# pennucci/PulsePortraiture

Hardware: AMD Instinct MI355X
Metric: subint_fits_per_sec (higher is better)
Workload: dtype f64

## Files before the change

### pulseportraiture_amd/csrc/pp_common.h

```cpp
#pragma once
#include <hip/hip_runtime.h>
#include <stdint.h>
#include <type_traits>

namespace pp {

#define PP_DCONST 4149.377593360996
#define PP_TWO_PI 6.283185307179586476925286766559
#define PP_LN10 2.302585092994045684017991454684

typedef double2 cplx;

__device__ __forceinline__ cplx cmul(cplx a, cplx b) {
    return make_double2(fma(a.x, b.x, -a.y * b.y), fma(a.x, b.y, a.y * b.x));
}
__device__ __forceinline__ cplx cmulc(cplx a, cplx b) {
    return make_double2(fma(a.x, b.x, a.y * b.y), fma(a.y, b.x, -a.x * b.y));
}
__device__ __forceinline__ cplx cadd(cplx a, cplx b) { return make_double2(a.x + b.x, a.y + b.y); }
__device__ __forceinline__ cplx csub(cplx a, cplx b) { return make_double2(a.x - b.x, a.y - b.y); }
__device__ __forceinline__ cplx cmul_mi(cplx a) { return make_double2(a.y, -a.x); }
__device__ __forceinline__ double cnorm(cplx a) { return fma(a.x, a.x, a.y * a.y); }

template <typename T>
__device__ __forceinline__ const T* as_global(const T* p) {
    typedef const T __attribute__((address_space(1)))* gp_t;
    return (const T*)(gp_t)(uintptr_t)p;
}

template <typename T>
__device__ __forceinline__ T load_uniform(const T* p) {
    typedef const T __attribute__((address_space(4)))* cp_t;
    return *(cp_t)(uintptr_t)p;
}

__device__ __forceinline__ double rn_pin(double r) { asm volatile("" : "+v"(r)); return r; }
__device__ __forceinline__ double mul_rn(double a, double b) { return rn_pin(a * b); }
__device__ __forceinline__ double add_rn(double a, double b) { return rn_pin(a + b); }
__device__ __forceinline__ double sub_rn(double a, double b) { return rn_pin(a - b); }

__device__ __forceinline__ double recip_ge1(double x) {
    double y = __builtin_amdgcn_rcp(x);
    y = fma(fma(-x, y, 1.0), y, y);
    y = fma(fma(-x, y, 1.0), y, y);
    return (x < 1e300) ? y : 0.0;
}

template <bool SC>
__device__ __forceinline__ double kconst(double v) {
    if (SC) asm volatile("" : "+s"(v));
    return v;
}
template <bool SC = false>
__device__ __forceinline__ void sincos_turns(double t, double* sn, double* cs) {
    const double q = rint(4.0 * t);
    const double y = fma(-0.25, q, t);
    const double u = y * y;
    double ps = kconst<SC>(0x1.aaec32af93359p-4);
    ps = fma(ps, u, kconst<SC>(-0x1.6fadb9f155744p-1));
    ps = fma(ps, u, kconst<SC>(0x1.e8f434d018d63p+1));
    ps = fma(ps, u, kconst<SC>(-0x1.e3074fde8871fp+3));
    ps = fma(ps, u, kconst<SC>(0x1.50783487ee782p+5));
    ps = fma(ps, u, kconst<SC>(-0x1.32d2cce62bd86p+6));
    ps = fma(ps, u, kconst<SC>(0x1.466bc6775aae2p+6));
    ps = fma(ps, u, kconst<SC>(-0x1.4abbce625be53p+5));
    ps = fma(ps, u, kconst<SC>(0x1.921fb54442d18p+2));
    const double s0 = ps * y;
    double pc = kconst<SC>(0x1.20c62c2f2d7f5p-2);
    pc = fma(pc, u, kconst<SC>(-0x1.b6e24f44b128fp+0));
    pc = fma(pc, u, kconst<SC>(0x1.f9d38a3763cc3p+2));
    pc = fma(pc, u, kconst<SC>(-0x1.a6d1f2a204a8cp+4));
    pc = fma(pc, u, kconst<SC>(0x1.e1f506891babbp+5));
    pc = fma(pc, u, kconst<SC>(-0x1.55d3c7e3cbffap+6));
    pc = fma(pc, u, kconst<SC>(0x1.03c1f081b5ac4p+6));
    pc = fma(pc, u, kconst<SC>(-0x1.3bd3cc9be45dep+4));
    const double c0 = fma(pc, u, 1.0);
    const int qi = (int)q;
    const bool odd = qi & 1;
    const double so = odd ? c0 : s0, co = odd ? s0 : c0;
    *sn = (qi & 2) ? -so : so;
    *cs = ((qi + 1) & 2) ? -co : co;
}

template <bool SC = false>
__device__ __forceinline__ cplx unit_phasor(double k, double phi) {
    double pfrac = phi - rint(phi);
    double prod = k * pfrac;
    double err = fma(k, pfrac, -prod);
    double r = (prod - rint(prod)) + err;
    double s, c;
    sincos_turns<SC>(r, &s, &c);
    return make_double2(c, s);
}

template <int W>
__device__ __forceinline__ double group_sum(double v) {
#pragma unroll
    for (int o = W / 2; o > 0; o >>= 1) v += __shfl_xor(v, o, 64);
    return v;
}
template <int W>
__device__ __forceinline__ double group_max(double v) {
#pragma unroll
    for (int o = W / 2; o > 0; o >>= 1) v = fmax(v, __shfl_xor(v, o, 64));
    return v;
}

__device__ __forceinline__ int wave_reduce16_index(int lane) { return (lane >> 2) & 15; }
template <int NS>
__device__ __forceinline__ double wave_reduce16(const double (&s)[NS], int lane) {
    double t8[8], t4[4], t2[2];
    const bool b5 = lane & 32, b4 = lane & 16, b3 = lane & 8, b2 = lane & 4;
#pragma unroll
    for (int j = 0; j < 8; ++j) {
        const double hi = (j + 8 < NS) ? s[j + 8] : 0.0;
        const double keep = b5 ? hi : s[j], send = b5 ? s[j] : hi;
        t8[j] = keep + __shfl_xor(send, 32, 64);
    }
#pragma unroll
    for (int j = 0; j < 4; ++j) {
        const double keep = b4 ? t8[j + 4] : t8[j], send = b4 ? t8[j] : t8[j + 4];
        t4[j] = keep + __shfl_xor(send, 16, 64);
    }
#pragma unroll
    for (int j = 0; j < 2; ++j) {
        const double keep = b3 ? t4[j + 2] : t4[j], send = b3 ? t4[j] : t4[j + 2];
        t2[j] = keep + __shfl_xor(send, 8, 64);
    }
    const double keep = b2 ? t2[1] : t2[0], send = b2 ? t2[0] : t2[1];
    double v = keep + __shfl_xor(send, 4, 64);
    v += __shfl_xor(v, 2, 64);
    v += __shfl_xor(v, 1, 64);
    return v;
}

template <int NS>
__device__ __forceinline__ double wave_reduce_lds(const double (&s)[NS], int lane, double* buf) {
    static_assert(NS <= 16, "one value per lane quad");
    const int wpos = (lane >> 4) * 17 + (lane & 15);
#pragma unroll
    for (int q = 0; q < NS; ++q) buf[q * 68 + wpos] = s[q];
    const int q = min(lane >> 2, NS - 1), part = lane & 3;
    const double* src = buf + q * 68 + part * 17;
    double v = 0.0;
#pragma unroll
    for (int t = 0; t < 16; ++t) v += src[t];
    v += __shfl_xor(v, 1, 64);
    v += __shfl_xor(v, 2, 64);
    return v;
}
#define PP_WRED_DOUBLES(NS) ((NS) * 68)

template <int NV>
__device__ inline void block_sum(double (&v)[NV], double* scratch) {
    const int lane = threadIdx.x & 63, wid = threadIdx.x >> 6, nw = blockDim.x >> 6;
#pragma unroll
    for (int i = 0; i < NV; ++i) v[i] = group_sum<64>(v[i]);
    __syncthreads();
    if (lane == 0) {
#pragma unroll
        for (int i = 0; i < NV; ++i) scratch[wid * NV + i] = v[i];
    }
    __syncthreads();
#pragma unroll
    for (int i = 0; i < NV; ++i) {
        double s = 0.0;
        for (int w = 0; w < nw; ++w) s += scratch[w * NV + i];
        v[i] = s;
    }
}

template <int NV, int C0>
__device__ __forceinline__ void wave_totals_to(const double (&v)[NV], int lane, double* dst) {
    constexpr int n = (NV - C0) < 16 ? (NV - C0) : 16;
    double part[n];
#pragma unroll
    for (int j = 0; j < n; ++j) part[j] = v[C0 + j];
    const double tot = wave_reduce16<n>(part, lane);
    if ((lane & 3) == 0 && (lane >> 2) < n) dst[C0 + (lane >> 2)] = tot;
    if constexpr (C0 + 16 < NV) wave_totals_to<NV, C0 + 16>(v, lane, dst);
}
// ... 57 lines not shown
```

### pulseportraiture_amd/csrc/pp_kernels.h

```cpp
#pragma once
#include "pp_fft.h"

namespace pp {

struct ModelFftArgs {
    const void* port;
    cplx* mft;
    double* msum;
    double* mmax;
    double* mdc;
    double* msq;
    const cplx* twB;
    int nchan;
};

struct TailArgs;
#define PP_TAIL_LDS_DOUBLES 2176
#define PP_TAIL_CACHE ((PP_TAIL_LDS_DOUBLES - 536) / 4)
__device__ void tail_work(const TailArgs* t, double* lds, int nlds, int tid, int max_tickets);

struct XspecArgs {
    const void* data;
    const cplx* const* mft;
    const cplx* mft0;
    const int* const* ktab;
    const int* kt0;
    const int* slot;
    cplx* X;
    double* sdraw;
    double* noise;
    const cplx* twB;
    int nsub, nchan, Kt;
    int Xs;
    const double* x0;
    const double* P;
    const double* nu_fit;
    const double* freqs; long long freqs_stride;
    double* csum0;
    double* tay;
    const double* ph0;
    const int* act;
    int cstep, coff, nchan_full;
    unsigned* ticket;
    unsigned ticket_base;
    int x_f32;
    const unsigned* mwords;
    const TailArgs* tail;
    int tail_nsub;
};

__device__ __forceinline__ void store_x(const XspecArgs& a, size_t row, int k, const cplx& x) {
    if (a.x_f32) reinterpret_cast<float2*>(a.X)[row * a.Xs + (k - 1)] = make_float2((float)x.x, (float)x.y);
    else a.X[row * a.Xs + (k - 1)] = x;
}

struct FitArgs {
    int nsub, nchan, nbin, M, Kt;
    int Xs;
    int flags[5];
    int log10_tau, option, is_toa, max_iter, scat;
    int method;
    const cplx* X;
    const cplx* const* mft;
    const double* const* msq;
    const double* const* msum;
    const int* const* ktab;
    const int* slot;
    const double* freqs; long long freqs_stride;
    const double* wts;
    const double* sdraw;
    const double* P;
    const double* nu_fit;
    const double* nu_out;
    const double* x0;
    SubState* st;
    double* csum;
    int ncs;
    double* tay;
    double* partial;
    int nchunk, cpc;
    int* nactive;
    double* o_params; double* o_errs; double* o_nu; double* o_cov;
    double* o_chi2; double* o_rchi2; double* o_snr; int* o_nfev; int* o_rc; int* o_npass;
    double* o_scales; double* o_scale_errs; double* o_csnr;
    double* o_f0; double* o_g0; double* o_H0;
    double* o_rec;
    const int* act;
    int nact, nchan_x, cstep, coff;
    double* mdl;
    int use_model;
    double model_tol;
    int model_bet;
    int recentre;
    double* x0w;
    int x_f32;
    const double* xstart;
    int nfev_shadow;
    int solve_cache;
    int tail_fused;
    int x_full;
};

__device__ __forceinline__ int sub_of(const int* act, int j) { return act ? act[j] : j; }

template <typename P>
__device__ __forceinline__ const P* uniform_ptr(const P* p) {
    const unsigned long long u = reinterpret_cast<unsigned long long>(p);
    const unsigned lo = (unsigned)__builtin_amdgcn_readfirstlane((int)(unsigned)u);
    const unsigned hi = (unsigned)__builtin_amdgcn_readfirstlane((int)(unsigned)(u >> 32));
    return as_global(reinterpret_cast<const P*>(((unsigned long long)hi << 32) | (unsigned long long)lo));
}

__device__ __forceinline__ bool channel_lookup(const XspecArgs& a, int ia, int n, int ne, int M, int& n_held,
                                               const cplx*& mrow, int& ktn) {
    if (!a.slot && n == n_held) return false;
    const cplx* m = as_global(a.slot ? a.mft[a.slot[ia]] : a.mft0) + (size_t)ne * M;
    const int k = a.ktab ? as_global(a.slot ? a.ktab[a.slot[ia]] : a.kt0)[ne] : a.Kt;
    mrow = uniform_ptr(m);
    ktn = __builtin_amdgcn_readfirstlane(k);
    n_held = n;
    return true;
}

template <int M, typename Tin>
__global__ __launch_bounds__(FftPlan<M>::T) void k_model_fft(ModelFftArgs a) {
    constexpr int T = FftPlan<M>::T;
    __shared__ cplx lds[FftPlan<M>::LDS_ELEMS];
    __shared__ double red[2 * (T / 64) + 2];
    const int tid = threadIdx.x;
    for (int n = blockIdx.x; n < a.nchan; n += gridDim.x) {
        const Tin* grow = reinterpret_cast<const Tin*>(a.port) + (size_t)n * (2 * M);
        fft_row<M, Tin>(lds, grow, a.twB, tid);
        double s = 0.0, mx = 0.0;
        for (int k = 1 + tid; k <= M; k += T) {
            const cplx d = rfft_harmonic<M>(lds, a.twB, k);
            a.mft[(size_t)n * M + (k - 1)] = d;
            const double p = cnorm(d);
            a.msq[(size_t)n * M + (k - 1)] = p;
            s += p;
            mx = fmax(mx, p);
        }
        s = group_sum<64>(s);
        mx = group_max<64>(mx);
        if (T > 64) {
            if ((tid & 63) == 0) { red[2 * (tid >> 6)] = s; red[2 * (tid >> 6) + 1] = mx; }
            __syncthreads();
            if (tid == 0) {
                s = 0.0; mx = 0.0;
                for (int w = 0; w < T / 64; ++w) { s += red[2 * w]; mx = fmax(mx, red[2 * w + 1]); }
            }
        }
        if (tid == 0) {
            a.msum[n] = s; a.mmax[n] = mx;
            const cplx z0 = lds[0];
            a.mdc[n] = z0.x + z0.y;
        }
        __syncthreads();
    }
}

__global__ void k_model_kcut(const cplx* mft, const double* mmax, int , int M, double eps2,
                             int* kt, int* kmax) {
    const int n = blockIdx.x;
    const double thr = eps2 * mmax[n];
    int last = 0;
    for (int k = 1 + threadIdx.x; k <= M; k += blockDim.x)
        if (cnorm(mft[(size_t)n * M + k - 1]) > thr) last = k;
    for (int o = 32; o > 0; o >>= 1) last = max(last, __shfl_xor(last, o, 64));
    if ((threadIdx.x & 63) == 0) {
        const int v = min(M, max(64, ((last + 63) / 64) * 64));
        kt[n] = v;
// ... 1021 lines not shown
    return rho > 0.15;
}

#define PP_FOR_N3(n_, EXPR)           \
    switch (n_) {                     \
        case 1: { constexpr int N_ = 1; EXPR; } break; \
        case 2: { constexpr int N_ = 2; EXPR; } break; \
        default: { constexpr int N_ = 3; EXPR; } break; \
    }
__device__ __forceinline__ double sel3(double v0, double v1, double v2, int k) { return k == 0 ? v0 : (k == 1 ? v1 : v2); }
template <int N>
__device__ __forceinline__ void gather_sub3(const double (&g)[3], const double (&H)[9], const int (&ix)[3], double (&gs)[N],
                                            double (&Hs)[N * N]) {
#pragma unroll
    for (int r = 0; r < N; ++r) {
        const int k = ix[r];
        gs[r] = sel3(g[0], g[1], g[2], k);
        const double r0 = sel3(H[0], H[3], H[6], k), r1 = sel3(H[1], H[4], H[7], k), r2 = sel3(H[2], H[5], H[8], k);
#pragma unroll
        for (int c = 0; c < N; ++c) Hs[r * N + c] = sel3(r0, r1, r2, ix[c]);
    }
}
template <int N>
__device__ __forceinline__ void scatter_sub3(const double (&p)[N], const int (&ix)[3], double (&p3)[3]) {
#pragma unroll
    for (int j = 0; j < 3; ++j) {
        p3[j] = 0.0;
#pragma unroll
        for (int r = 0; r < N; ++r) if (ix[r] == j) p3[j] = p[r];
    }
}
template <int N>
__device__ __forceinline__ void tr_propose_scipy3(double f, const double (&g)[3], const double (&H)[9], const int (&ix)[3],
                                                  double radius, double (&p3)[3], int& hits, double& pred) {
    double gs[N], Hs[N * N], p[N];
    gather_sub3<N>(g, H, ix, gs, Hs);
    tr_cg_steihaug_scipy<N>(f, gs, Hs, radius, p, &hits);
    pred = f - tr_model_value<N>(f, gs, Hs, p);
    scatter_sub3<N>(p, ix, p3);
}
template <int N>
__device__ __forceinline__ bool newton_propose3(const double (&g)[3], const double (&H)[9], const int (&ix)[3], double (&p3)[3],
                                                double& pred) {
    double gs[N], Hs[N * N], p[N], mg[N], Hp[N];
    gather_sub3<N>(g, H, ix, gs, Hs);
#pragma unroll
    for (int r = 0; r < N; ++r) mg[r] = -gs[r];
    if (!chol_solve<N>(Hs, mg, p)) return false;
#pragma unroll
    for (int r = 0; r < N; ++r) Hp[r] = vdot<N>(Hs + r * N, p);
    pred = -(vdot<N>(gs, p) + 0.5 * vdot<N>(p, Hp));
    scatter_sub3<N>(p, ix, p3);
    return true;
}

__global__ __launch_bounds__(256) void k_eval_moments(FitArgs a) {
    constexpr int LPC = 16;
    const int jx = blockIdx.x, i = sub_of(a.act, jx), chunk = blockIdx.y;
    const SubState& st = a.st[i];
    const int tid = threadIdx.x, g = tid / LPC, l = tid % LPC;
    const double phi = st.xe[0], DM = st.xe[1], GM = st.xe[2];
    const double P = a.P[i];
    const double nuDM = a.nu_fit[i * 3], nuGM = a.nu_fit[i * 3 + 1];
    const double* freqs = a.freqs + (size_t)i * a.freqs_stride;
    const double* wts = a.wts + (size_t)i * a.nchan;
    const int* ktv = a.ktab ? as_global(a.ktab[a.slot ? a.slot[i] : 0]) : nullptr;
    double* tay = a.tay;
    const size_t row0 = (size_t)i * a.nchan;
    const int n0 = chunk * a.cpc, n1 = min(n0 + a.cpc, a.nchan_x);
    const int src = ((tid & 63) & ~(LPC - 1)) | (LPC - 1);
    for (int nn = n0 + g; nn < n1; nn += 256 / LPC) {
        const int n = a.coff + nn * a.cstep;
        const double w = wts[n];
        double p1, p2;
        phase_geom(freqs[n], P, nuDM, nuGM, p1, p2);
        const double phin = phi + DM * p1 + GM * p2;
        cplx e0 = unit_phasor((double)(l + 1), phin);
        const cplx w1 = make_double2(__shfl(e0.x, src, 64), __shfl(e0.y, src, 64));
        const cplx w2 = cmul(w1, w1), w3 = cmul(w2, w1), w4 = cmul(w2, w2);
        const cplx* xrow = a.X + ((size_t)jx * a.nchan_x + nn) * a.Xs;
        const int ktn = ktv ? ktv[n] : a.Kt;
        double s[PP_TSTRIDE];
#pragma unroll
        for (int j = 0; j < PP_TSTRIDE; ++j) s[j] = 0.0;
        double k = (double)(l + 1);
        if (w != 0.0) {
#pragma unroll 1
            for (int jj = l; jj < ktn; jj += 4 * LPC) {
                const cplx zero = make_double2(0.0, 0.0);
                cplx xv[4];
                xv[0] = xrow[jj];
                xv[1] = (jj + LPC < ktn) ? xrow[jj + LPC] : zero;
                xv[2] = (jj + 2 * LPC < ktn) ? xrow[jj + 2 * LPC] : zero;
                xv[3] = (jj + 3 * LPC < ktn) ? xrow[jj + 3 * LPC] : zero;
                cplx ev[4];
                ev[0] = e0; ev[1] = cmul(e0, w1); ev[2] = cmul(e0, w2); ev[3] = cmul(e0, w3);
#pragma unroll
                for (int q = 0; q < 4; ++q) {
                    const cplx z = cmul(xv[q], ev[q]);
                    const double kap = PP_TWO_PI * (k + (double)(q * LPC));
                    const double kap2 = kap * kap;
                    double ur = z.x, ui = z.y * kap;
#pragma unroll
                    for (int j = 0; j <= PP_TJ; j += 2) {
                        s[j] += ur;
                        ur *= kap2;
                        if (j + 1 <= PP_TJ) { s[j + 1] += ui; ui *= kap2; }
                    }
                    static_assert(PP_TJ % 2 == 0, "PP_TJ must be even");
                    double pw = kap;
#pragma unroll
                    for (int j = 0; j < PP_TJ / 2; ++j) pw *= kap2;
                    s[PP_TJ + 1] = fma(pw, fabs(xv[q].x) + fabs(xv[q].y), s[PP_TJ + 1]);
                }
                e0 = cmul(e0, w4);
                k += 4.0 * LPC;
            }
        }
#pragma unroll
        for (int j = 0; j < PP_TSTRIDE; ++j) {
            double v = group_sum<LPC>(s[j]);
            if (j <= PP_TJ && ((j & 3) == 1 || (j & 3) == 2)) v = -v;
            if (l == (j % LPC)) tay[tay_idx(row0 + n, j)] = v;
        }
    }
}

__device__ __forceinline__ void taylor_load(const double* tay, size_t row, double (&t)[PP_TSTRIDE]) {
    static_assert(PP_TSTRIDE % 2 == 0, "rows of the Taylor model are read in pairs");
    const double* tg = tay + tay_idx(row, 0);
#pragma unroll
    for (int j = 0; j < PP_TSTRIDE / 2; ++j) {
        const double2 v = *reinterpret_cast<const double2*>(tg + j * PP_TAY_PAIR_STRIDE);
        t[2 * j] = v.x; t[2 * j + 1] = v.y;
    }
}
__device__ __forceinline__ void taylor_shift_reg(const double (&t)[PP_TSTRIDE], double d, double& A0, double& A1,
                                                 double& A2);
__device__ __forceinline__ void taylor_shift_reg(const double (&t)[PP_TSTRIDE], double d, double& A0, double& A1,
                                                 double& A2) {
    double a0 = 0.0, a1 = 0.0, a2 = 0.0;
#pragma unroll
    for (int j = PP_TJ; j >= 0; --j) {
        a0 = fma(a0, d * (1.0 / (double)(j + 1)), t[j]);
        if (j >= 1) a1 = fma(a1, d * (1.0 / (double)j), t[j]);
        if (j >= 2) a2 = fma(a2, d * (1.0 / (double)(j - 1)), t[j]);
    }
    A0 = a0; A1 = a1; A2 = a2;
}

#define PP_SOLVE_CACHE_MAX 4096
constexpr int PP_SOLVE_PF = 2;
constexpr int PP_TAYLOR_WAVES = 2;
template <int NV, int NVMAX, int NT, int NVW, typename F>
__device__ __forceinline__ void vblock_sum(double (&out)[NV], double* scratch, int& flip, double* mx, int tid, F&& accumulate) {
    static_assert(NV <= NVMAX, "scratch sized for NVMAX values");
    constexpr int NWV = NT / 64, RT = NT / NVW;
    const int lane = tid & 63, rw = tid >> 6;
    double* buf = scratch + flip * NWV * (NVMAX + 1);
    flip ^= 1;
    auto one_wave = [&](const int vw) __attribute__((always_inline)) {
#pragma unroll
        for (int j = 0; j < NV; ++j) out[j] = 0.0;
        double m = 0.0;
        accumulate(lane + 64 * vw, out, m);
        wave_totals_to<NV, 0>(out, lane, buf + vw * (NV + 1));
        if (mx) {
            m = group_max<64>(m);
            if (lane == 0) buf[vw * (NV + 1) + NV] = m;
        }
    };
    if constexpr (NVW == 1) one_wave(rw);
    else {
#pragma unroll 1
        for (int k = 0; k < NVW; ++k) one_wave(rw + (RT / 64) * k);
    }
    __syncthreads();
#pragma unroll
    for (int i = 0; i < NV; ++i) out[i] = 0.0;
#pragma unroll 1
    for (int w = 0; w < NWV; ++w) {
#pragma unroll
        for (int i = 0; i < NV; ++i) out[i] += buf[w * (NV + 1) + i];
    }
    if (mx) {
        double m = buf[NV];
#pragma unroll 1
        for (int w = 1; w < NWV; ++w) m = fmax(m, buf[w * (NV + 1) + NV]);
        *mx = m;
    }
}

template <int NT, int PF, int NVW>
__device__ __forceinline__ void taylor_solve_body(const FitArgs& a, const int i, const int tid, double* scratch, double* inv_lds) {
    constexpr int RT = NT / NVW;
    static_assert(NT % 64 == 0 && RT % 64 == 0 && NT % RT == 0, "whole waves");
    SubState& st = a.st[i];
    if (st.done) return;
    int flip = 0;
    const double P = a.P[i];
    const double nuDM = a.nu_fit[i * 3], nuGM = a.nu_fit[i * 3 + 1];
    const double* freqs = a.freqs + (size_t)i * a.freqs_stride;
    const double* wts = a.wts + (size_t)i * a.nchan;
    const double* msum = as_global(a.msum[a.slot ? a.slot[i] : 0]);
    const double* tay = a.tay;
    const size_t row0 = (size_t)i * a.nchan;
    const int* fl = a.flags;
    int ix[3] = {0, 0, 0}, nf = 0;
#pragma unroll
    for (int j = 0; j < 3; ++j)
        if (fl[j]) {
            if (nf == 0) ix[0] = j; else if (nf == 1) ix[1] = j; else ix[2] = j;
            ++nf;
        }
    const int ncache = a.solve_cache;
    double *inv_w = inv_lds, *inv_p1 = inv_lds + ncache, *inv_p2 = inv_lds + 2 * ncache, *inv_S = inv_lds + 3 * ncache;
    {
        const int nc = min(a.nchan, ncache);
#pragma unroll 4
        for (int n = tid; n < nc; n += RT) {
            double p1, p2;
            phase_geom(freqs[n], P, nuDM, nuGM, p1, p2);
            inv_w[n] = wts[n]; inv_p1[n] = p1; inv_p2[n] = p2; inv_S[n] = msum[n];
        }
        __syncthreads();
    }
    auto chan_inv = [&](int n, double& w, double& p1, double& p2, double& S0) {
        if (n < ncache) { w = inv_w[n]; p1 = inv_p1[n]; p2 = inv_p2[n]; S0 = inv_S[n]; }
        else { w = wts[n]; phase_geom(freqs[n], P, nuDM, nuGM, p1, p2); S0 = msum[n]; }
    };
    auto for_channels = [&](const int vt, auto&& body) {
        if constexpr (PF == 0) {
            for (int n = vt; n < a.nchan; n += NT) {
                double t[PP_TSTRIDE];
                taylor_load(tay, row0 + n, t);
                body(n, t);
            }
        } else {
            double buf[PF ? PF : 1][PP_TSTRIDE];
#pragma unroll
            for (int d = 0; d < PF; ++d)
                if (vt + d * NT < a.nchan) taylor_load(tay, row0 + vt + d * NT, buf[d]);
            for (int n0 = vt; n0 < a.nchan; n0 += PF * NT) {
#pragma unroll
                for (int d = 0; d < PF; ++d) {
                    const int n = n0 + d * NT;
                    if (n < a.nchan) {
                        double t[PP_TSTRIDE];
#pragma unroll
                        for (int j = 0; j < PP_TSTRIDE; ++j) t[j] = buf[d][j];
                        if (n + PF * NT < a.nchan) taylor_load(tay, row0 + n + PF * NT, buf[d]);
                        body(n, t);
                    }
                }
            }
        }
    };
    auto for_channels_at_origin = [&](const int vt, auto&& body) {
        constexpr int U = 4;
        for (int n0 = vt; n0 < a.nchan; n0 += U * NT) {
            double2 h[U][2];
#pragma unroll
            for (int d = 0; d < U; ++d)
                if (n0 + d * NT < a.nchan) {
                    const double* tg = tay + tay_idx(row0 + n0 + d * NT, 0);
                    h[d][0] = *reinterpret_cast<const double2*>(tg);
                    h[d][1] = *reinterpret_cast<const double2*>(tg + PP_TAY_PAIR_STRIDE);
                }
#pragma unroll
            for (int d = 0; d < U; ++d)
                if (n0 + d * NT < a.nchan) body(n0 + d * NT, h[d][0].x, h[d][0].y, h[d][1].x);
        }
    };
    auto evalm = [&](const double* dx, double& f, double* g, double* H, bool at_origin = false) -> double {
        double acc[10];
        double dmax = 0.0;
        vblock_sum<10, 10, NT, NVW>(acc, scratch, flip, &dmax, tid, [&](const int vt, double (&ac)[10], double& dm) __attribute__((always_inline)) {
            auto add = [&](double w, double p1, double p2, double S0, double A0, double A1, double A2) {
                const bool in = (w != 0.0);
                const double r = A0 / S0;
                const double F = in ? -w * A0 * r : 0.0, Gp = in ? -2.0 * w * r * A1 : 0.0;
                const double Lpp = in ? -2.0 * w * (A1 * A1 / S0 + r * A2) : 0.0;
                ac[0] += F;
                ac[1] += Gp; ac[2] += Gp * p1; ac[3] += Gp * p2;
                ac[4] += Lpp; ac[5] += Lpp * p1; ac[6] += Lpp * p2;
                ac[7] += Lpp * p1 * p1; ac[8] += Lpp * p1 * p2; ac[9] += Lpp * p2 * p2;
            };
            if (at_origin)
                for_channels_at_origin(vt, [&](int n, double A0, double A1, double A2) {
                    double w, p1, p2, S0;
                    chan_inv(n, w, p1, p2, S0);
                    add(w, p1, p2, S0, A0, A1, A2);
                });
            else
                for_channels(vt, [&](int n, const double (&t)[PP_TSTRIDE]) {
                    double w, p1, p2, S0;
                    chan_inv(n, w, p1, p2, S0);
                    const double d = dx[0] + dx[1] * p1 + dx[2] * p2;
                    dm = fmax(dm, (w != 0.0) ? fabs(d) : 0.0);
                    double A0, A1, A2;
                    taylor_shift_reg(t, d, A0, A1, A2);
                    add(w, p1, p2, S0, A0, A1, A2);
                });
        });
        f = acc[0];
        g[0] = fl[0] ? acc[1] : 0.0; g[1] = fl[1] ? acc[2] : 0.0; g[2] = fl[2] ? acc[3] : 0.0;
        const double hh[3][3] = {{acc[4], acc[5], acc[6]}, {acc[5], acc[7], acc[8]}, {acc[6], acc[8], acc[9]}};
#pragma unroll
        for (int r_ = 0; r_ < 3; ++r_)
#pragma unroll
            for (int c_ = 0; c_ < 3; ++c_) H[r_ * 3 + c_] = (fl[r_] && fl[c_]) ? hh[r_][c_] : 0.0;
        return dmax;
    };
    double dx[3] = {0.0, 0.0, 0.0};
    const bool off_centre = (a.xstart != nullptr) && st.recentred == 0;
    if (off_centre)
#pragma unroll
        for (int j = 0; j < 3; ++j) dx[j] = fl[j] ? a.xstart[i * 5 + j] - st.xe[j] : 0.0;
    const double dx0[3] = {dx[0], dx[1], dx[2]};
    double f, g[3], H[9];
    bool ok = true;
    int it = 0, nfev = 1;
    double dpath = evalm(dx, f, g, H, !off_centre);
    if (tid == 0 && st.recentred == 0) {
        st.f0 = f;
#pragma unroll
        for (int j = 0; j < 5; ++j) st.g0[j] = j < 3 ? g[j] : 0.0;
#pragma unroll
        for (int r_ = 0; r_ < 5; ++r_)
#pragma unroll
            for (int c_ = 0; c_ < 5; ++c_) st.H0[r_ * 5 + c_] = (r_ < 3 && c_ < 3) ? H[r_ * 3 + c_] : 0.0;
    }
    if (!isfinite(f)) ok = false;
    if (ok && a.method == 0) {
        double radius = 1.0;
        double xa[3], xla[3], xld[3] = {dx0[0], dx0[1], dx0[2]};
#pragma unroll
        for (int j = 0; j < 3; ++j) { xa[j] = off_centre ? (fl[j] ? a.xstart[i * 5 + j] : st.xe[j]) : st.xe[j]; xla[j] = xa[j]; }
        double f2 = f, g2[3] = {g[0], g[1], g[2]}, H2[9];
#pragma unroll
        for (int j = 0; j < 9; ++j) H2[j] = H[j];
        for (;;) {
            double p3[3], pred = 0.0;
            int hits = 0;
            PP_FOR_N3(nf, (tr_propose_scipy3<N_>(f, g, H, ix, radius, p3, hits, pred)));
            double xta[3], xt[3];
#pragma unroll
            for (int j = 0; j < 3; ++j) { xta[j] = fl[j] ? xa[j] + p3[j] : xa[j]; xt[j] = fl[j] ? dx[j] + p3[j] : dx[j]; }
            if (a.nfev_shadow >= 2)
#pragma unroll
                for (int j = 0; j < 3; ++j) xt[j] = xta[j] - st.xe[j];
            const bool shadow = a.nfev_shadow > 0 || (a.nfev_shadow < 0 && nf == 1);
            const bool cached = shadow ? (xta[0] == xla[0] && xta[1] == xla[1] && xta[2] == xla[2])
                                              : (xt[0] == xld[0] && xt[1] == xld[1] && xt[2] == xld[2]);
            if (!(pred > 0.0)) {
                if (!cached) ++nfev;
                break;
            }
            if (!cached) {
                dpath = fmax(dpath, evalm(xt, f2, g2, H2));
#pragma unroll
                for (int j = 0; j < 3; ++j) { xla[j] = xta[j]; xld[j] = xt[j]; }
                ++nfev;
            }
            bool finite = isfinite(f2);
#pragma unroll
            for (int j = 0; j < 3; ++j) finite = finite && isfinite(g2[j]);
#if defined(PP_TAYLOR_TRACE) && PP_TAYLOR_TRACE >= 3
            if (tid == 0)
                printf("tay it %2d f %.17g f_new %.17g actual %.3e pred %.3e rho %.3f radius %.3e hits %d cached %d\n", it, f, f2,
                       f - f2, pred, (f - f2) / pred, radius, hits, (int)cached);
#endif
            if (tr_scipy_accept(f, f2, pred, hits, finite, &radius)) {
#pragma unroll
                for (int j = 0; j < 3; ++j) { dx[j] = xt[j]; xa[j] = xta[j]; }
                f = f2;
#pragma unroll
                for (int j = 0; j < 3; ++j) g[j] = g2[j];
#pragma unroll
                for (int j = 0; j < 9; ++j) H[j] = H2[j];
            }
            ++it;
            if (it >= a.max_iter || !(radius > 1e-300)) {
#ifdef PP_TAYLOR_TRACE
                if (tid == 0) printf("taylor %d: iteration limit it %d radius %.3e\n", i, it, radius);
#endif
                ok = false; break;
            }
        }
    } else if (ok) {
        double fprev = INFINITY;
        for (it = 0; it < 24; ++it) {
            if (it > 0) { dpath = fmax(dpath, evalm(dx, f, g, H)); ++nfev; }
            if (!isfinite(f)) { ok = false; break; }
            double p3[3], pred = 0.0;
            bool solved = false;
            PP_FOR_N3(nf, (solved = newton_propose3<N_>(g, H, ix, p3, pred)));
            if (!solved) { ok = false; break; }
            if (f > fprev + 1e-9 * fabs(fprev)) { ok = false; break; }
            fprev = f;
#pragma unroll
            for (int j = 0; j < 3; ++j) if (fl[j]) dx[j] += p3[j];
            if (!(pred > 64.0 * 2.220446049250313e-16 * fabs(f))) break;
        }
        if (it >= 24) ok = false;
    }
    const int buf = 1 - st.cur;
    if (ok) {
        double* csum = a.csum + ((size_t)buf * a.nsub + i) * a.nchan * a.ncs;
        double ev[4];
        double jf = 1.0;
        for (int j = 2; j <= PP_TJ; ++j) jf *= (double)j;
        vblock_sum<4, 10, NT, NVW>(ev, scratch, flip, nullptr, tid, [&](const int vt, double (&e4)[4], double&) __attribute__((always_inline)) {
            for_channels(vt, [&](int n, const double (&t)[PP_TSTRIDE]) {
                double w, p1, p2, S0;
                chan_inv(n, w, p1, p2, S0);
                const double d = dx[0] + dx[1] * p1 + dx[2] * p2;
                double A0, A1, A2;
                taylor_shift_reg(t, d, A0, A1, A2);
                csum[(size_t)n * 3] = A0; csum[(size_t)n * 3 + 1] = A1; csum[(size_t)n * 3 + 2] = A2;
                if (w == 0.0) return;
                e4[3] += -w * A0 * A0 / S0;
                const double d2 = d * d, d4 = d2 * d2, d10 = d4 * d4 * d2;
                static_assert(PP_TJ == 10, "remainder power written for order 10");
                const double e1 = t[PP_TJ + 1] * d10 / jf;
                const double r = fabs(t[0] / S0) + 1e-300;
                const double ge = 2.0 * w * r * e1 * 1.5;
                e4[0] += ge; e4[1] += ge * fabs(p1); e4[2] += ge * fabs(p2);
            });
        });
        const double tol[3] = {1e-13, 1e-11, 1e-8};
#pragma unroll
        for (int j = 0; j < 3; ++j)
            if (fl[j]) {
                const double hjj = fabs(H[j * 3 + j]);
#if defined(PP_TAYLOR_TRACE) && PP_TAYLOR_TRACE >= 2
                if (tid == 0 && j == 0) printf("tmargin %d %.4e %.4e\n", i, ev[j] / (tol[j] * hjj), dpath);
#endif
                if (!(ev[j] <= tol[j] * hjj)) {
#ifdef PP_TAYLOR_TRACE
                    if (tid == 0) printf("taylor %d: certificate %d: err %.3e > tol %.3e (dpath %.3e, it %d) x0 %.9f %.9f dx %.3e %.3e f %.10e\n", i, j, ev[j], tol[j] * hjj, dpath, it, st.xe[0], st.xe[1], dx[0], dx[1], f);
// ... 674 lines not shown
```

### pulseportraiture_amd/csrc/pp_tail.h

```cpp
#pragma once
#include "pp_kernels.h"
#include "pp_extra.h"
#include "pp_xspec1024r.h"

namespace pp {

struct RefTailArgs {
    int on;
    int ncc;
    const cplx* part;
    const double* delta;
    const double* wsum;
    const unsigned* mws;
    const cplx* mspec;
    int mstride;
    FpsArgs fps;
    double* xs;
    double* seed_phase;
};
struct TailArgs {
    FitArgs fa;
    unsigned ticket, done;
    int nsub;
    int solve_nt, solve_pf;
    int fin_nt;
    RefTailArgs rs;
};

__device__ __forceinline__ void refseed_ticket(const RefTailArgs& r, const int nsub, const int i, const int tid, double* lds) {
    constexpr int M = 1024;
    static_assert(128 + 2 * M <= PP_TAIL_LDS_DOUBLES, "the fit's cross-spectrum in the carrying kernel's image");
    cplx* X = reinterpret_cast<cplx*>(lds + 128);
    {
        const double delta_i = r.delta[i], wsum_i = r.wsum[i];
        const double inv = wsum_i > 0.0 ? 1.0 / wsum_i : 0.0;
        cplx s[RS_NACC];
#pragma unroll
        for (int q = 0; q < RS_NACC; ++q) s[q] = make_double2(0.0, 0.0);
        const cplx* base = r.part + (size_t)i * r.ncc * RS_NACC * 64 + tid;
#pragma unroll 2
        for (int cc = 0; cc < r.ncc; ++cc) {
            if (r.mws && r.mws[(size_t)cc * nsub + i] == 0u) continue;
            cplx v[RS_NACC];
#pragma unroll
            for (int q = 0; q < RS_NACC; ++q)
                v[q] = (q < RS_NREG || tid == 0) ? base[((size_t)cc * RS_NACC + q) * 64] : make_double2(0.0, 0.0);
#pragma unroll
            for (int q = 0; q < RS_NACC; ++q) { s[q].x += v[q].x; s[q].y += v[q].y; }
        }
        const int lam = fftq_lambda(tid);
        auto put = [&](const int k, cplx t) __attribute__((always_inline)) {
            const cplx rot = unit_phasor((double)k, -delta_i);
            t = cmul(t, rot);
            t.x *= inv; t.y *= inv;
            if (k == M) t.y = 0.0;
            X[k - 1] = t;
        };
#pragma unroll
        for (int q = 0; q < 7; ++q) put(lam != 0 ? lam + 64 * q : 64 * (q + 1), s[q]);
#pragma unroll
        for (int q = 7; q < RS_NREG; ++q) put(lam + 64 * (12 + q - 7), s[q]);
        if (lam == 0) put(M, s[RS_NREG]);
#pragma unroll
        for (int kd = 7; kd < 12; ++kd) {
            const int k = lam + 64 * kd;
            if (k > 448) X[k - 1] = make_double2(0.0, 0.0);
        }
    }
    __syncthreads();
    const cplx* m = r.mspec + (size_t)i * r.mstride;
    auto dv = [&](const int k) __attribute__((always_inline)) { return X[k - 1]; };
    fps_body<4>(r.fps, i, tid, M, dv, m, X, lds, nullptr, nullptr);
    __syncthreads();
    if (tid == 0) refseed_start_one(r.fps.out7, i, r.xs, r.seed_phase);
    __syncthreads();
}

__device__ __noinline__ void tail_work(const TailArgs* t, double* lds, int nlds, int tid, int max_tickets) {
    TailArgs* tw = const_cast<TailArgs*>(t);
    const int nsub = t->nsub;
    for (int round = 0; round < max_tickets; ++round) {
        unsigned tk = 0;
        if (tid == 0) tk = atomicAdd(&tw->ticket, 1u);
        tk = (unsigned)__builtin_amdgcn_readfirstlane((int)tk);
        if (tk >= (unsigned)nsub) return;
        const FitArgs& a = t->fa;
        const int i = (int)tk;
        double* scratch = lds;
        double* sh = lds + 528;
        double* inv = lds + 536;
        (void)nlds;
        if (t->rs.on) refseed_ticket(t->rs, nsub, i, tid, lds);
        const int snt = t->solve_nt, spf = t->solve_pf, fnt = t->fin_nt;
        if (snt == 64) taylor_solve_body<64, PP_SOLVE_PF, 1>(a, i, tid, scratch, inv);
        else if (snt == 128) taylor_solve_body<128, PP_SOLVE_PF, 2>(a, i, tid, scratch, inv);
        else if (snt == 512) taylor_solve_body<512, PP_SOLVE_PF, 8>(a, i, tid, scratch, inv);
        else if (spf == 0) taylor_solve_body<256, 0, 4>(a, i, tid, scratch, inv);
        else taylor_solve_body<256, PP_SOLVE_PF, 4>(a, i, tid, scratch, inv);
        __syncthreads();
        if (fnt == 64) finalize_body<8, 64, 1>(a, i, tid, scratch, sh);
        else if (fnt == 128) finalize_body<0, 128, 2>(a, i, tid, scratch, sh);
        else if (fnt == 512) finalize_body<0, 512, 8>(a, i, tid, scratch, sh);
        else finalize_body<0, 256, 4>(a, i, tid, scratch, sh);
        __syncthreads();
        if (tid == 0) {
            __threadfence();
            const unsigned d = atomicAdd(&tw->done, 1u);
            if (d + 1u == (unsigned)nsub) {
                __threadfence();
                a.o_npass[a.nsub] = atomicAdd(a.nactive, 0);
            }
        }
    }
}

}
```

Measured before the change: 76000.

## Stage Taylor coefficient rows through an LDS tile with coalesced prefetch in tail solve

In the tail solve, each wave now loads 64 channels' Taylor coefficient rows with coalesced double2 global reads, writes them to an LDS tile and reads them back transposed per lane, separated only by wave barriers. Per-channel weight, frequency and msum values are prefetched one tile ahead. The goal is to replace strided per-lane row loads with coalesced traffic and to hide global latency. In exchange the tile takes LDS space from the inverse cache, the spf==0 path is dropped, and the at-origin case now goes through the generic loop.

```diff
diff --git a/pulseportraiture_amd/csrc/pp_common.h b/pulseportraiture_amd/csrc/pp_common.h
--- a/pulseportraiture_amd/csrc/pp_common.h
+++ b/pulseportraiture_amd/csrc/pp_common.h
@@ -27,6 +27,10 @@
     typedef const T __attribute__((address_space(1)))* gp_t;
     return (const T*)(gp_t)(uintptr_t)p;
 }
+
+typedef double pp_dv2 __attribute__((ext_vector_type(2)));
+typedef pp_dv2 __attribute__((address_space(3))) pp_lds_dv2;
+__device__ __forceinline__ pp_lds_dv2* as_lds_pairs(double* p) { return (pp_lds_dv2*)(unsigned)(uintptr_t)p; }
 
 template <typename T>
 __device__ __forceinline__ T load_uniform(const T* p) {
diff --git a/pulseportraiture_amd/csrc/pp_kernels.h b/pulseportraiture_amd/csrc/pp_kernels.h
--- a/pulseportraiture_amd/csrc/pp_kernels.h
+++ b/pulseportraiture_amd/csrc/pp_kernels.h
@@ -16,7 +16,8 @@
 
 struct TailArgs;
 #define PP_TAIL_LDS_DOUBLES 2176
-#define PP_TAIL_CACHE ((PP_TAIL_LDS_DOUBLES - 536) / 4)
+#define PP_TAIL_TILE_DOUBLES 768
+#define PP_TAIL_CACHE ((PP_TAIL_LDS_DOUBLES - 536 - PP_TAIL_TILE_DOUBLES) / 4)
 __device__ void tail_work(const TailArgs* t, double* lds, int nlds, int tid, int max_tickets);
 
 struct XspecArgs {
@@ -1344,6 +1345,7 @@
 #define PP_SOLVE_CACHE_MAX 4096
 constexpr int PP_SOLVE_PF = 2;
 constexpr int PP_TAYLOR_WAVES = 2;
+constexpr int PP_TILE_AHEAD = 1;
 template <int NV, int NVMAX, int NT, int NVW, typename F>
 __device__ __forceinline__ void vblock_sum(double (&out)[NV], double* scratch, int& flip, double* mx, int tid, F&& accumulate) {
     static_assert(NV <= NVMAX, "scratch sized for NVMAX values");
@@ -1383,10 +1385,12 @@
     }
 }
 
-template <int NT, int PF, int NVW>
-__device__ __forceinline__ void taylor_solve_body(const FitArgs& a, const int i, const int tid, double* scratch, double* inv_lds) {
+template <int NT, int PF, int NVW, bool TILE = false>
+__device__ __forceinline__ void taylor_solve_body(const FitArgs& a, const int i, const int tid, double* scratch, double* inv_lds,
+                                                  double* tile = nullptr) {
     constexpr int RT = NT / NVW;
     static_assert(NT % 64 == 0 && RT % 64 == 0 && NT % RT == 0, "whole waves");
+    static_assert(!TILE || RT == 64, "the tile goes through LDS without a barrier: one real wave");
     SubState& st = a.st[i];
     if (st.done) return;
     int flip = 0;
@@ -1417,12 +1421,71 @@
         }
         __syncthreads();
     }
+    double pre_w = 0.0, pre_f = 0.0, pre_S = 0.0;
     auto chan_inv = [&](int n, double& w, double& p1, double& p2, double& S0) {
         if (n < ncache) { w = inv_w[n]; p1 = inv_p1[n]; p2 = inv_p2[n]; S0 = inv_S[n]; }
+        else if constexpr (TILE) { w = pre_w; phase_geom(pre_f, P, nuDM, nuGM, p1, p2); S0 = pre_S; }
         else { w = wts[n]; phase_geom(freqs[n], P, nuDM, nuGM, p1, p2); S0 = msum[n]; }
     };
     auto for_channels = [&](const int vt, auto&& body) {
-        if constexpr (PF == 0) {
+        if constexpr (TILE) {
+            static_assert(PP_TSTRIDE == 12 && PP_TAY_PAIR_STRIDE == 2 && PP_TAIL_TILE_DOUBLES == 64 * PP_TSTRIDE,
+                          "a tile is 64 whole rows of six coefficient pairs");
+            constexpr int TD = PP_TILE_AHEAD, NP = PP_TSTRIDE / 2;
+            const int lane = vt & 63, c00 = __builtin_amdgcn_readfirstlane(vt - lane);
+            const int nchan = a.nchan;
+            pp_lds_dv2* const tl = as_lds_pairs(tile);
+            const double2* const g0 = as_global(reinterpret_cast<const double2*>(tay + tay_idx(row0, 0)));
+            const double *const gw = as_global(wts), *const gf = as_global(freqs), *const gS = as_global(msum);
+            double2 nx[TD][NP];
+            double ni[TD][3];
+            auto fetch = [&](const int c0, double2 (&v)[NP], double (&iv)[3]) {
+                if (c0 + 64 <= nchan) {
+                    const double2* const g = g0 + (c0 * NP + lane);
+#pragma unroll
+                    for (int j = 0; j < NP; ++j) v[j] = g[64 * j];
+                    iv[0] = gw[c0 + lane]; iv[1] = gf[c0 + lane]; iv[2] = gS[c0 + lane];
+                } else {
+                    const int last = nchan * NP - 1;
+#pragma unroll
+                    for (int j = 0; j < NP; ++j) v[j] = g0[min(c0 * NP + lane + 64 * j, last)];
+                    const int nn = min(c0 + lane, nchan - 1);
+                    iv[0] = gw[nn]; iv[1] = gf[nn]; iv[2] = gS[nn];
+                }
+            };
+#pragma unroll
+            for (int d = 0; d < TD; ++d)
+                if (c00 + d * NT < nchan) fetch(c00 + d * NT, nx[d], ni[d]);
+            for (int c1 = c00; c1 < nchan; c1 += TD * NT) {
+#pragma unroll
+                for (int d = 0; d < TD; ++d) {
+                    const int c0 = c1 + d * NT;
+                    if (c0 < nchan) {
+#pragma unroll
+                        for (int j = 0; j < NP; ++j) {
+                            pp_dv2 v;
+                            v.x = nx[d][j].x; v.y = nx[d][j].y;
+                            tl[lane + 64 * j] = v;
+                        }
+                        pre_w = ni[d][0]; pre_f = ni[d][1]; pre_S = ni[d][2];
+                        if (c0 + TD * NT < nchan) fetch(c0 + TD * NT, nx[d], ni[d]);
+                        __builtin_amdgcn_fence(__ATOMIC_RELEASE, "wavefront");
+                        __builtin_amdgcn_wave_barrier();
+                        __builtin_amdgcn_fence(__ATOMIC_ACQUIRE, "wavefront");
+                        double t[PP_TSTRIDE];
+#pragma unroll
+                        for (int j = 0; j < NP; ++j) {
+                            const pp_dv2 v = tl[lane * NP + j];
+                            t[2 * j] = v.x; t[2 * j + 1] = v.y;
+                        }
+                        __builtin_amdgcn_fence(__ATOMIC_RELEASE, "wavefront");
+                        __builtin_amdgcn_wave_barrier();
+                        __builtin_amdgcn_fence(__ATOMIC_ACQUIRE, "wavefront");
+                        if (c0 + lane < nchan) body(c0 + lane, t);
+                    }
+                }
+            }
+        } else if constexpr (PF == 0) {
             for (int n = vt; n < a.nchan; n += NT) {
                 double t[PP_TSTRIDE];
                 taylor_load(tay, row0 + n, t);
@@ -1478,7 +1541,13 @@
                 ac[4] += Lpp; ac[5] += Lpp * p1; ac[6] += Lpp * p2;
                 ac[7] += Lpp * p1 * p1; ac[8] += Lpp * p1 * p2; ac[9] += Lpp * p2 * p2;
             };
-            if (at_origin)
+            if (TILE && at_origin)
+                for_channels(vt, [&](int n, const double (&t)[PP_TSTRIDE]) {
+                    double w, p1, p2, S0;
+                    chan_inv(n, w, p1, p2, S0);
+                    add(w, p1, p2, S0, t[0], t[1], t[2]);
+                });
+            else if (at_origin)
                 for_channels_at_origin(vt, [&](int n, double A0, double A1, double A2) {
                     double w, p1, p2, S0;
                     chan_inv(n, w, p1, p2, S0);
diff --git a/pulseportraiture_amd/csrc/pp_tail.h b/pulseportraiture_amd/csrc/pp_tail.h
--- a/pulseportraiture_amd/csrc/pp_tail.h
+++ b/pulseportraiture_amd/csrc/pp_tail.h
@@ -88,15 +88,17 @@
         const int i = (int)tk;
         double* scratch = lds;
         double* sh = lds + 528;
-        double* inv = lds + 536;
+        double* tile = lds + 536;
+        double* inv = lds + 536 + PP_TAIL_TILE_DOUBLES;
+        static_assert(536 + PP_TAIL_TILE_DOUBLES + 4 * PP_TAIL_CACHE <= PP_TAIL_LDS_DOUBLES, "tail_work's layout");
         (void)nlds;
         if (t->rs.on) refseed_ticket(t->rs, nsub, i, tid, lds);
         const int snt = t->solve_nt, spf = t->solve_pf, fnt = t->fin_nt;
-        if (snt == 64) taylor_solve_body<64, PP_SOLVE_PF, 1>(a, i, tid, scratch, inv);
-        else if (snt == 128) taylor_solve_body<128, PP_SOLVE_PF, 2>(a, i, tid, scratch, inv);
-        else if (snt == 512) taylor_solve_body<512, PP_SOLVE_PF, 8>(a, i, tid, scratch, inv);
-        else if (spf == 0) taylor_solve_body<256, 0, 4>(a, i, tid, scratch, inv);
-        else taylor_solve_body<256, PP_SOLVE_PF, 4>(a, i, tid, scratch, inv);
+        (void)spf;
+        if (snt == 64) taylor_solve_body<64, PP_SOLVE_PF, 1, true>(a, i, tid, scratch, inv, tile);
+        else if (snt == 128) taylor_solve_body<128, PP_SOLVE_PF, 2, true>(a, i, tid, scratch, inv, tile);
+        else if (snt == 512) taylor_solve_body<512, PP_SOLVE_PF, 8, true>(a, i, tid, scratch, inv, tile);
+        else taylor_solve_body<256, PP_SOLVE_PF, 4, true>(a, i, tid, scratch, inv, tile);
         __syncthreads();
         if (fnt == 64) finalize_body<8, 64, 1>(a, i, tid, scratch, sh);
         else if (fnt == 128) finalize_body<0, 128, 2>(a, i, tid, scratch, sh);
```

After: 76090, median of 2. About the same (+0.1%).
